# zc402/video-classification

Measured on AMD Instinct MI355X. Metric: clips/sec SlowFast-R50 8x8, 32x224^2 bf16 training step, higher is better.
Workload: dtype bf16

## Files before the change

### video-classification_amd/csrc/optim_misc.hip

```cpp
#include <string.h>

#include "sfk_common.h"

namespace {

__global__ void adam_step_inc_kernel(int64_t* step) { step[0] += 1; }

template <typename S>
__global__ __launch_bounds__(256) void adam_kernel(float* __restrict__ p, const float* __restrict__ g,
                                                   float* __restrict__ m, float* __restrict__ v, int64_t count,
                                                   float lr, float b1, float b2, float eps, float gscale,
                                                   const int64_t* step, S* __restrict__ shadow) {
  __shared__ float bc[2];
  if (threadIdx.x == 0) {
    const double t = (double)step[0];
    bc[0] = (float)(1.0 - pow((double)b1, t));
    bc[1] = (float)(1.0 - pow((double)b2, t));
  }
  __syncthreads();
  const float step_size = lr / bc[0];
  const float inv_sqrt_bc2 = 1.f / sqrtf(bc[1]);
  for (int64_t i = ((int64_t)blockIdx.x * 256 + threadIdx.x) * 4; i < count; i += (int64_t)gridDim.x * 1024) {
    if (i + 3 < count) {
      float4 pv = *reinterpret_cast<float4*>(p + i);
      const float4 gv = *reinterpret_cast<const float4*>(g + i);
      float4 mv = *reinterpret_cast<float4*>(m + i);
      float4 vv = *reinterpret_cast<float4*>(v + i);
      float* pp = reinterpret_cast<float*>(&pv);
      const float* gp = reinterpret_cast<const float*>(&gv);
      float* mp = reinterpret_cast<float*>(&mv);
      float* vp = reinterpret_cast<float*>(&vv);
#pragma unroll
      for (int j = 0; j < 4; ++j) {
        const float gj = gp[j] * gscale;
        mp[j] = b1 * mp[j] + (1.f - b1) * gj;
        vp[j] = b2 * vp[j] + (1.f - b2) * gj * gj;
        pp[j] -= step_size * mp[j] / (sqrtf(vp[j]) * inv_sqrt_bc2 + eps);
      }
      *reinterpret_cast<float4*>(p + i) = pv;
      *reinterpret_cast<float4*>(m + i) = mv;
      *reinterpret_cast<float4*>(v + i) = vv;
      if (shadow) {
#pragma unroll
        for (int j = 0; j < 4; ++j) shadow[i + j] = (S)pp[j];
      }
    } else {
      for (int64_t e = i; e < count; ++e) {
        const float gj = g[e] * gscale;
        m[e] = b1 * m[e] + (1.f - b1) * gj;
        v[e] = b2 * v[e] + (1.f - b2) * gj * gj;
        p[e] -= step_size * m[e] / (sqrtf(v[e]) * inv_sqrt_bc2 + eps);
        if (shadow) shadow[e] = (S)p[e];
      }
    }
  }
}

template <typename S, typename D>
__global__ __launch_bounds__(256) void cast_kernel(const S* __restrict__ src, D* __restrict__ dst, int64_t count) {
  for (int64_t i = (int64_t)blockIdx.x * 256 + threadIdx.x; i < count; i += (int64_t)gridDim.x * 256)
    dst[i] = (D)(float)src[i];
}

template <typename S, typename D>
__global__ __launch_bounds__(256) void filter_transpose_kernel(const S* __restrict__ src, D* __restrict__ dst,
                                                               int cout, int wtaps, int cin) {
  const int64_t total = (int64_t)cout * wtaps * cin;
  for (int64_t i = (int64_t)blockIdx.x * 256 + threadIdx.x; i < total; i += (int64_t)gridDim.x * 256) {
    const int co = (int)(i % cout);
    const int64_t r = i / cout;
    const int wi = (int)(r % wtaps);
    const int ci = (int)(r / wtaps);
    dst[i] = (D)(float)src[((int64_t)co * wtaps + wi) * cin + ci];
  }
}

template <typename D>
__global__ __launch_bounds__(256) void filter_refresh_kernel(const float* __restrict__ master, D* __restrict__ s,
                                                             D* __restrict__ st, const sfk_filter_ent* __restrict__ table,
                                                             int n) {
  __shared__ float tile[32][33];
  int lo = 0, hi = n - 1;
  const int b = blockIdx.x;
  while (lo < hi) {
    const int mid = (lo + hi + 1) >> 1;
    if (table[mid].first_block <= b) lo = mid; else hi = mid - 1;
  }
  const sfk_filter_ent e = table[lo];
  const int tiles_ci = (e.cin + 31) / 32;
  int lb = b - e.first_block;
  const int tap = lb % e.wtaps;
  lb /= e.wtaps;
  const int ci0 = (lb % tiles_ci) * 32, co0 = (lb / tiles_ci) * 32;
  const int tx = threadIdx.x & 31, ty = threadIdx.x >> 5;
#pragma unroll
  for (int i = 0; i < 4; ++i) {
    const int co = co0 + ty + 8 * i, ci = ci0 + tx;
    float v = 0.f;
    if (co < e.cout && ci < e.cin) {
      const int64_t idx = e.off + ((int64_t)co * e.wtaps + tap) * e.cin + ci;
      v = master[idx];
      if (s) s[idx] = (D)v;
    }
    tile[ty + 8 * i][tx] = v;
  }
  if (!st || !e.transpose) return;
  __syncthreads();
#pragma unroll
  for (int i = 0; i < 4; ++i) {
    const int ci = ci0 + ty + 8 * i, co = co0 + tx;
    if (co < e.cout && ci < e.cin) st[e.off + ((int64_t)ci * e.wtaps + tap) * e.cout + co] = (D)tile[tx][ty + 8 * i];
  }
}

inline unsigned grid_for(int64_t total, int per_thread = 1) {
  int64_t b = (total + 256ll * per_thread - 1) / (256ll * per_thread);
  if (b > 16384) b = 16384;
  if (b < 1) b = 1;
  return (unsigned)b;
}

}

extern "C" int sfk_adam(float* p, const float* g, float* m, float* v, int64_t count, float lr, float beta1,
                        float beta2, float eps, float grad_scale, int64_t* step, void* shadow,
                        int32_t shadow_dtype, sfk_stream_t stream) {
  if (!p || !g || !m || !v || !step || count <= 0) return SFK_ERR_INVALID;
  if ((((uintptr_t)p) | ((uintptr_t)g) | ((uintptr_t)m) | ((uintptr_t)v)) & 15) return SFK_ERR_UNSUPPORTED;
  hipStream_t s = static_cast<hipStream_t>(stream);
  hipLaunchKernelGGL(adam_step_inc_kernel, dim3(1), dim3(1), 0, s, step);
  const dim3 grid(grid_for(count, 4)), blk(256);
  if (shadow && shadow_dtype == SFK_BF16)
    hipLaunchKernelGGL(adam_kernel<bf16_t>, grid, blk, 0, s, p, g, m, v, count, lr, beta1, beta2, eps, grad_scale, step, static_cast<bf16_t*>(shadow));
  else
    hipLaunchKernelGGL(adam_kernel<float>, grid, blk, 0, s, p, g, m, v, count, lr, beta1, beta2, eps, grad_scale, step, static_cast<float*>(shadow));
  SFK_CHECK_LAUNCH();
  return SFK_OK;
}


static inline bool dtype_ok(int d) { return d == SFK_F32 || d == SFK_BF16; }

extern "C" int sfk_filter_transpose(const void* src, int32_t src_dtype, void* dst, int32_t dst_dtype, int32_t cout,
                                    int32_t wtaps, int32_t cin, sfk_stream_t stream) {
  if (!src || !dst || cout <= 0 || wtaps <= 0 || cin <= 0 || !dtype_ok(src_dtype) || !dtype_ok(dst_dtype))
    return SFK_ERR_INVALID;
  hipStream_t s = static_cast<hipStream_t>(stream);
  const int64_t total = (int64_t)cout * wtaps * cin;
  if (src_dtype == SFK_F32 && dst_dtype == SFK_F32)
    hipLaunchKernelGGL((filter_transpose_kernel<float, float>), dim3(grid_for(total)), dim3(256), 0, s, (const float*)src, (float*)dst, cout, wtaps, cin);
  else if (src_dtype == SFK_F32 && dst_dtype == SFK_BF16)
    hipLaunchKernelGGL((filter_transpose_kernel<float, bf16_t>), dim3(grid_for(total)), dim3(256), 0, s, (const float*)src, (bf16_t*)dst, cout, wtaps, cin);
  else if (src_dtype == SFK_BF16 && dst_dtype == SFK_F32)
    hipLaunchKernelGGL((filter_transpose_kernel<bf16_t, float>), dim3(grid_for(total)), dim3(256), 0, s, (const bf16_t*)src, (float*)dst, cout, wtaps, cin);
  else
    hipLaunchKernelGGL((filter_transpose_kernel<bf16_t, bf16_t>), dim3(grid_for(total)), dim3(256), 0, s, (const bf16_t*)src, (bf16_t*)dst, cout, wtaps, cin);
  SFK_CHECK_LAUNCH();
  return SFK_OK;
}

extern "C" int sfk_filter_refresh(const float* master, void* s, void* st, int32_t dtype, const sfk_filter_ent* table,
                                  int32_t n_layers, int32_t total_blocks, sfk_stream_t stream) {
  if (!master || (!s && !st) || !table || n_layers <= 0 || total_blocks <= 0 || !dtype_ok(dtype)) return SFK_ERR_INVALID;
  hipStream_t hs = static_cast<hipStream_t>(stream);
  if (dtype == SFK_BF16)
    hipLaunchKernelGGL((filter_refresh_kernel<bf16_t>), dim3((unsigned)total_blocks), dim3(256), 0, hs, master, (bf16_t*)s, (bf16_t*)st, table, n_layers);
  else
    hipLaunchKernelGGL((filter_refresh_kernel<float>), dim3((unsigned)total_blocks), dim3(256), 0, hs, master, (float*)s, (float*)st, table, n_layers);
  SFK_CHECK_LAUNCH();
  return SFK_OK;
}

extern "C" int sfk_cast(const void* src, int32_t src_dtype, void* dst, int32_t dst_dtype, int64_t count,
                        sfk_stream_t stream) {
  if (!src || !dst || count <= 0 || !dtype_ok(src_dtype) || !dtype_ok(dst_dtype)) return SFK_ERR_INVALID;
  hipStream_t s = static_cast<hipStream_t>(stream);
  if (src_dtype == SFK_F32 && dst_dtype == SFK_F32)
    hipLaunchKernelGGL((cast_kernel<float, float>), dim3(grid_for(count, 4)), dim3(256), 0, s, (const float*)src, (float*)dst, count);
  else if (src_dtype == SFK_F32 && dst_dtype == SFK_BF16)
    hipLaunchKernelGGL((cast_kernel<float, bf16_t>), dim3(grid_for(count, 4)), dim3(256), 0, s, (const float*)src, (bf16_t*)dst, count);
  else if (src_dtype == SFK_BF16 && dst_dtype == SFK_F32)
    hipLaunchKernelGGL((cast_kernel<bf16_t, float>), dim3(grid_for(count, 4)), dim3(256), 0, s, (const bf16_t*)src, (float*)dst, count);
  else
    hipLaunchKernelGGL((cast_kernel<bf16_t, bf16_t>), dim3(grid_for(count, 4)), dim3(256), 0, s, (const bf16_t*)src, (bf16_t*)dst, count);
  SFK_CHECK_LAUNCH();
  return SFK_OK;
}

extern "C" int sfk_fill_zero(void* p, size_t bytes, sfk_stream_t stream) {
  if (!p) return SFK_ERR_INVALID;
  if (bytes == 0) return SFK_OK;
  return hipMemsetAsync(p, 0, bytes, static_cast<hipStream_t>(stream)) == hipSuccess ? SFK_OK : SFK_ERR_LAUNCH;
}

namespace {
constexpr sfk_tuning kDefaults = {(uint32_t)sizeof(sfk_tuning), 5, 0, 1, 192, 256, 1, 7, 1024, 0, 48, 150, 1, 1ll << 20, 3, 512, 1, 16, 1, 3, 3};
sfk_tuning g_tuning = kDefaults;
bool g_tuning_set = false;
}
const sfk_tuning& sfk_tune() { return g_tuning; }

extern "C" int sfk_default_tuning(sfk_tuning* out) {
  if (!out || out->struct_size != sizeof(sfk_tuning)) return SFK_ERR_INVALID;
  *out = kDefaults;
  return SFK_OK;
}

extern "C" int sfk_get_tuning(sfk_tuning* out) {
  if (!out || out->struct_size != sizeof(sfk_tuning)) return SFK_ERR_INVALID;
  *out = g_tuning;
  return SFK_OK;
}

extern "C" int sfk_init(const sfk_tuning* t) {
  sfk_tuning want = kDefaults;
  if (t) {
    if (t->struct_size != sizeof(sfk_tuning)) return SFK_ERR_INVALID;
    want = *t;
  }
  if (want.bn_parts < 1 || want.wgrad_target_8w < 1 || want.wgrad_target_4w < 1 || want.pool_blocks < 1 ||
      want.igemm_short_k < 0)
    return SFK_ERR_INVALID;
  if (g_tuning_set) return memcmp(&want, &g_tuning, sizeof(want)) == 0 ? SFK_OK : SFK_ERR_INVALID;
  g_tuning = want;
  g_tuning_set = true;
  return SFK_OK;
}

extern "C" int sfk_abi_version(void) { return SFK_ABI_VERSION; }

extern "C" const char* sfk_status_string(int status) {
  switch (status) {
    case SFK_OK: return "ok";
    case SFK_ERR_INVALID: return "invalid argument";
    case SFK_ERR_UNSUPPORTED: return "unsupported shape or alignment";
    case SFK_ERR_LAUNCH: return "kernel launch failed";
    default: return "unknown status";
  }
}
```

### video-classification_amd/csrc/stem_conv.hip

```cpp
#include "sfk_common.h"

namespace {

constexpr int TS = 16;
constexpr int PR = 2 * TS + 5;
constexpr int PC = 40;
constexpr int KH = 7;

struct StemK {
  const void* src;
  int64_t sn, sc, st, sh, sw;
  int cin, t_in, h_in, w_in;
  const int32_t* t_index;
  int t_log;
  int kt, pt;
  int krows;
  int kp;
  int planes;
  int cout;
  int ho, wo, t_out;
  int tiles_h, tiles_w;
  FastDiv dtw, dth, dt, d7, dcin, dpc;
  const void* w;
  void* y;
// ... 815 lines not shown
  const int tid = threadIdx.x, lane = tid & 63, l15 = lane & 15, g = lane >> 4;
  const int wave = __builtin_amdgcn_readfirstlane(tid >> 6);
  bf16_t* yp = static_cast<bf16_t*>(k.y);
  auto a_off = [](int r, int sg) { return r * 64 + ((sg ^ ((4 - ((r >> 2) & 3)) & 3)) << 4); };
  const int perm_g = ((g & 1) << 1) | (g >> 1);
  {
    const bf16_t* wp = static_cast<const bf16_t*>(k.w);
    for (int e = tid; e < NCH * 64; e += 256) {
      const int ch = e >> 6, row = (e >> 2) & 15, gg = e & 3;
      const int cf = ch / CPF, c6 = ch % CPF;
      const int co = 16 * cf + row;
      const int kh = (c6 & 1) * 4 + (((gg & 1) << 1) | (gg >> 1)), ci = c6 >> 1;
      bf16x8 v;
#pragma unroll
      for (int i = 0; i < 8; ++i) v[i] = (bf16_t)0.f;
      if (co < k.cout && kh < KH) {
        const bf16x8 wv = *reinterpret_cast<const bf16x8*>(wp + (int64_t)co * k.kp + (ci * KH + kh) * 8);
#pragma unroll
        for (int i = 1; i < 8; ++i) v[i] = wv[i - 1];
      }
      *reinterpret_cast<bf16x8*>(amat + ch * 1024 + a_off(row, gg)) = v;
    }
  }
  __syncthreads();
  bf16x8 afr[NCH];
  {
    const int a_lane = a_off(l15, g);
#pragma unroll
    for (int ch = 0; ch < NCH; ++ch) {
      afr[ch] = *reinterpret_cast<const bf16x8*>(amat + ch * 1024 + a_lane);
      asm volatile("" : "+v"(afr[ch]));
    }
  }
  H2Stage<CIN> stg;
  stg.init(k, tid);
  uint4 xra[4], xrb[4];
  const __amdgpu_buffer_rsrc_t srs = sfk_make_rsrc(k.src, k.src_bytes);
  const __amdgpu_buffer_rsrc_t srs0 = sfk_make_rsrc(k.src, 0);
  const int b_lane = (4 * wave + perm_g) * F2_PITCH + (2 * l15 + 4) * 2;
  const int tpairs = (k.t_log + 1) / 2;
  const int tiles_h2 = (k.ho + H2_ROWS - 1) / H2_ROWS;
  H2Unit u;
  const int lb = (gridDim.x & 7) == 0 ? (int)((blockIdx.x & 7) * (gridDim.x >> 3) + (blockIdx.x >> 3)) : (int)blockIdx.x;
  for (int unit = lb; unit < nunits; unit += gridDim.x) {
    u.set(k, unit, pairs_per_unit, tchunks, tiles_h2, tpairs);
    const int n = u.n, p0 = u.p0, p1 = u.p1;
    const int ho0 = u.th2 * H2_ROWS, wo0 = u.tw * TS;
    stg.unit(k, ho0, wo0);
    const int fbase = 2 * p0;
    if (tid < 2 * (p1 - p0)) {
      const int F = fbase + tid;
      int f = (F >= 0 && F < k.t_log) ? F : -1;
      if (f >= 0 && k.t_index) f = k.t_index[f];
      fidx[tid] = (f >= 0 && f < k.t_in) ? f : -1;
    }
    __syncthreads();
    auto frame_of = [&](int F) { return __builtin_amdgcn_readfirstlane(fidx[F - fbase]); };
    stg.fetch(k, xra, srs, srs0, n, frame_of(2 * p0), frame_of(2 * p0 + 1));
    stg.stage(pb, xra);
    if (p0 + 1 < p1) stg.fetch(k, xrb, srs, srs0, n, frame_of(2 * (p0 + 1)), frame_of(2 * (p0 + 1) + 1));
    __syncthreads();
    float s1[NCF][4], s2[NCF][4];
#pragma unroll
    for (int cf = 0; cf < NCF; ++cf)
#pragma unroll
      for (int r = 0; r < 4; ++r) s1[cf][r] = s2[cf][r] = 0.f;
    auto pair_iter = [&](const int m, const int cur, uint4 (&xf)[4], const uint4 (&xs)[4]) __attribute__((always_inline)) {
      if (m + 2 < p1) stg.fetch(k, xf, srs, srs0, n, frame_of(2 * (m + 2)), frame_of(2 * (m + 2) + 1));
#pragma unroll
      for (int par = 0; par < 2; ++par) {
        const int to = 2 * m + par;
        if (to >= k.t_out) continue;
        const char* bb = pb + (cur * 2 + par) * SLOT + b_lane;
        f32x4 acc[NCF][2];
#pragma unroll
        for (int cf = 0; cf < NCF; ++cf) acc[cf][0] = acc[cf][1] = f32x4{0.f, 0.f, 0.f, 0.f};
#pragma unroll
        for (int c6 = 0; c6 < CPF; ++c6) {
          bf16x8 bv[2];
#pragma unroll
          for (int j = 0; j < 2; ++j) {
            const uint32_t* q = reinterpret_cast<const uint32_t*>(bb + (c6 >> 1) * H2_PLANE + (2 * j + 4 * (c6 & 1)) * F2_PITCH);
            uint4 t4 = make_uint4(q[0], q[1], q[2], q[3]);
            bv[j] = *reinterpret_cast<const bf16x8*>(&t4);
          }
#pragma unroll
          for (int cf = 0; cf < NCF; ++cf) {
            acc[cf][0] = __builtin_amdgcn_mfma_f32_16x16x32_bf16(afr[cf * CPF + c6], bv[0], acc[cf][0], 0, 0, 0);
            acc[cf][1] = __builtin_amdgcn_mfma_f32_16x16x32_bf16(afr[cf * CPF + c6], bv[1], acc[cf][1], 0, 0, 0);
          }
        }
        const int wo = wo0 + l15;
#pragma unroll
        for (int j = 0; j < 2; ++j) {
          const int ho = ho0 + 2 * wave + j;
          const bool pok = ho < k.ho && wo < k.wo;
          if (pok) {
#pragma unroll
            for (int cf = 0; cf < NCF; ++cf)
#pragma unroll
              for (int r = 0; r < 4; ++r) { s1[cf][r] += acc[cf][j][r]; s2[cf][r] += acc[cf][j][r] * acc[cf][j][r]; }
          }
          bf16_t* pix = yp + ((((int64_t)n * k.t_out + to) * k.ho + ho) * k.wo + wo) * k.yld + k.yoff;
#pragma unroll
          for (int cp = 0; cp < NCF; cp += 2) {
            float v[8] = {acc[cp][j][0], acc[cp][j][1], acc[cp][j][2], acc[cp][j][3],
                          acc[cp + 1][j][0], acc[cp + 1][j][1], acc[cp + 1][j][2], acc[cp + 1][j][3]};
#pragma unroll
            for (int e = 0; e < 4; ++e) stem_swap16(v[e], v[4 + e]);
            const int co = 16 * cp + 16 * (g & 1) + 8 * (g >> 1);
            if (pok && co < k.cout) {
              bf16x8 o;
#pragma unroll
              for (int e = 0; e < 8; ++e) o[e] = (bf16_t)v[e];
              *reinterpret_cast<bf16x8*>(pix + co) = o;
            }
          }
        }
      }
      if (m + 1 < p1) stg.stage(pb + (cur ^ 1) * 2 * SLOT, xs);
      __syncthreads();
    };
    for (int m = p0;;) {
      pair_iter(m, 0, xra, xrb);
      if (++m >= p1) break;
      pair_iter(m, 1, xrb, xra);
      if (++m >= p1) break;
    }
    if (k.stats) {
#pragma unroll
      for (int cf = 0; cf < NCF; ++cf)
#pragma unroll
        for (int r = 0; r < 4; ++r) {
          const float a = stem_row16_sum(s1[cf][r]), c = stem_row16_sum(s2[cf][r]);
          if (l15 == 15) {
            red[(wave * 64 + 16 * cf + 4 * g + r) * 2 + 0] = a;
            red[(wave * 64 + 16 * cf + 4 * g + r) * 2 + 1] = c;
          }
        }
      __syncthreads();
      const int half = u.th2 & 1, th = u.th2 >> 1;
      const bool alone = (u.th2 | 1) >= tiles_h2;
      const int nfr = min(2 * p1, k.t_out) - 2 * p0;
      for (int e = tid; e < nfr * k.cout; e += 256) {
        const int fr = e / k.cout, co = e - fr * k.cout;
        if (!alone && (fr & 1) != half) continue;
        float a1 = 0.f, a2 = 0.f;
        if (fr == half) {
#pragma unroll
          for (int w_ = 0; w_ < 4; ++w_) { a1 += red[(w_ * 64 + co) * 2]; a2 += red[(w_ * 64 + co) * 2 + 1]; }
        }
        const int64_t trow = (((int64_t)n * k.t_out + 2 * p0 + fr) * k.tiles_h + th) * k.tiles_w + u.tw;
        k.stats[(trow * k.cout + co) * 2 + 0] = a1;
        k.stats[(trow * k.cout + co) * 2 + 1] = a2;
      }
    }
  }
}

constexpr int V2_PC = 56;
constexpr int V2_PR = 38;
constexpr int V2_CH = 6;
constexpr int V2_DROW = 128;

__device__ __forceinline__ int v2_swz(int px) { return ((px >> 1) & 1) | (((px >> 3) & 1) << 1); }

template <int CIN>
__global__ __launch_bounds__(256, 2) void stem_wgrad_v2_kernel(const StemK k) {
  constexpr int PLANE = V2_PR * V2_PC * 2;
  constexpr int NXC = (CIN * V2_PR * V2_CH + 255) / 256;
  constexpr int NDC = 5;
  __shared__ __attribute__((aligned(16))) char smem[CIN * PLANE + 256 * V2_DROW];
  char* patch = smem;
  char* dyt = smem + CIN * PLANE;
  const int tid = threadIdx.x, lane = tid & 63, l15 = lane & 15, g = lane >> 4;
  const int wave = __builtin_amdgcn_readfirstlane(tid >> 6);
  const int lb = (gridDim.x & 7) == 0 ? (int)((blockIdx.x & 7) * (gridDim.x >> 3) + (blockIdx.x >> 3)) : (int)blockIdx.x;
  const int item0 = lb * k.tiles_per_block;
  const int item1 = min(item0 + k.tiles_per_block, k.ntiles);
  if (item0 >= item1) return;
  const bf16_t* src = static_cast<const bf16_t*>(k.src);
  const bf16_t* dyp = static_cast<const bf16_t*>(k.y);

  int x_ci[NXC], x_r[NXC], x_j[NXC];
#pragma unroll
  for (int i = 0; i < NXC; ++i) {
    const int e = tid + 256 * i;
    x_ci[i] = e / (V2_PR * V2_CH);
    const int rem = e % (V2_PR * V2_CH);
    x_r[i] = rem / V2_CH;
    x_j[i] = rem % V2_CH;
    if (e >= CIN * V2_PR * V2_CH) x_ci[i] = -1;
  }
  uint4 xr[NXC], dr[NDC];
  const __amdgpu_buffer_rsrc_t srs = sfk_make_rsrc(k.src, k.src_bytes);
  const __amdgpu_buffer_rsrc_t yrs = sfk_make_rsrc(k.y, k.y_bytes);
  const __amdgpu_buffer_rsrc_t srs0 = sfk_make_rsrc(k.src, 0);
  const __amdgpu_buffer_rsrc_t yrs0 = sfk_make_rsrc(k.y, 0);
  int x_chan[NXC];
#pragma unroll
  for (int i = 0; i < NXC; ++i) x_chan[i] = x_ci[i] < 0 ? 0 : (int)(x_ci[i] * k.sc * 2);
  auto fetch = [&](int item) {
    int n, tf, ho0, wo0;
    tile_coords(k, item, n, tf, ho0, wo0);
    int frame = k.t_index ? __builtin_amdgcn_readfirstlane(k.t_index[tf]) : tf;
    const bool fok = frame >= 0 && frame < k.t_in;
    const uint32_t xso = fok ? (uint32_t)(((int64_t)n * k.sn + (int64_t)frame * k.st) * 2) : 0u;
#pragma unroll
    for (int i = 0; i < NXC; ++i) {
      const int hi = 2 * ho0 - 3 + x_r[i], wi = 2 * wo0 - 8 + 8 * x_j[i];
      const bool ok = x_ci[i] >= 0 && (unsigned)hi < (unsigned)k.h_in && wi >= 0 && wi + 8 <= k.w_in;
      const uint32_t vo = ok ? (uint32_t)(x_chan[i] + (hi * (int)k.sh + wi) * 2) : 0x80000000u;
      const u32x4 v = __builtin_amdgcn_raw_buffer_load_b128(fok ? srs : srs0, (int)vo, (int)xso, 0);
      xr[i] = make_uint4(v[0], v[1], v[2], v[3]);
    }
    const int ho = ho0 + (tid >> 4), wo = wo0 + (tid & 15);
    const bool pok = ho < k.ho && wo < k.wo;
    const uint32_t yvo = pok ? (uint32_t)(((ho * k.wo + wo) * k.yld + k.yoff) * 2) : 0x80000000u;
    const int64_t fstride = (int64_t)k.ho * k.wo * k.yld * 2;
#pragma unroll
    for (int f = 0; f < NDC; ++f) {
      const int to = tf + k.pt - f;
      const bool ok = f < k.kt && to >= 0 && to < k.t_out;
      const uint32_t yso = ok ? (uint32_t)(((int64_t)n * k.t_out + to) * fstride) : 0u;
      const u32x4 v = __builtin_amdgcn_raw_buffer_load_b128(ok ? yrs : yrs0, (int)yvo, (int)yso, 0);
      dr[f] = make_uint4(v[0], v[1], v[2], v[3]);
    }
  };
  auto stage = [&]() {
#pragma unroll
    for (int i = 0; i < NXC; ++i)
      if (x_ci[i] >= 0)
        *reinterpret_cast<uint4*>(patch + x_ci[i] * PLANE + x_r[i] * (V2_PC * 2) + x_j[i] * 16) = xr[i];
    const int sw = v2_swz(tid);
#pragma unroll
    for (int f = 0; f < NDC; ++f)
      *reinterpret_cast<uint4*>(dyt + tid * V2_DROW + (((f >> 1) ^ sw) << 5) + (f & 1) * 16) = dr[f];
    *reinterpret_cast<uint4*>(dyt + tid * V2_DROW + ((2 ^ sw) << 5) + 16) = make_uint4(0, 0, 0, 0);
  };

  const int khh = l15 >> 3, kw = l15 & 7;
  const uint32_t sel = (kw & 1) ? 0x05040100u : 0x07060302u;
  const int cbe = (kw & 1) ? 5 + kw : 4 + kw;
  const int b_lane = ((g >> 1) * 2 + 2 * wave + khh) * (V2_PC * 2) + (2 * (g & 1) * 8 + cbe) * 2;
  const int q = l15 >> 2, p4 = lane & 3;
  int a_lane[3];
#pragma unroll
  for (int i = 0; i < 3; ++i) {
    const int row = 8 * g + q;
    a_lane[i] = row * V2_DROW + ((i ^ v2_swz(row)) << 5) + p4 * 8;
  }
  f32x4 acc[CIN][3];
#pragma unroll
  for (int c = 0; c < CIN; ++c)
#pragma unroll
    for (int i = 0; i < 3; ++i) acc[c][i] = f32x4{0.f, 0.f, 0.f, 0.f};

  fetch(item0);
  for (int item = item0; item < item1; ++item) {
    __syncthreads();
    stage();
    __syncthreads();
    if (item + 1 < item1) fetch(item + 1);
#pragma unroll
    for (int s = 0; s < 8; ++s) {
      bf16x8 a[3];
#pragma unroll
      for (int i = 0; i < 3; ++i) {
        const char* ap = dyt + s * 32 * V2_DROW + a_lane[i];
        const bf16x4 lo = __builtin_amdgcn_ds_read_tr16_b64_v4bf16((lds_bf16x4*)(ap));
        const bf16x4 hi = __builtin_amdgcn_ds_read_tr16_b64_v4bf16((lds_bf16x4*)(ap + 4 * V2_DROW));
        a[i][0] = lo[0]; a[i][1] = lo[1]; a[i][2] = lo[2]; a[i][3] = lo[3];
        a[i][4] = hi[0]; a[i][5] = hi[1]; a[i][6] = hi[2]; a[i][7] = hi[3];
      }
#pragma unroll
      for (int c = 0; c < CIN; ++c) {
        const uint32_t* bp = reinterpret_cast<const uint32_t*>(patch + c * PLANE + s * 4 * (V2_PC * 2) + b_lane);
        uint32_t d[8];
#pragma unroll
        for (int e = 0; e < 8; ++e) d[e] = bp[e];
        uint4 bv;
        bv.x = __builtin_amdgcn_perm(d[1], d[0], sel);
        bv.y = __builtin_amdgcn_perm(d[3], d[2], sel);
        bv.z = __builtin_amdgcn_perm(d[5], d[4], sel);
        bv.w = __builtin_amdgcn_perm(d[7], d[6], sel);
        const bf16x8 b = *reinterpret_cast<const bf16x8*>(&bv);
#pragma unroll
        for (int i = 0; i < 3; ++i) acc[c][i] = __builtin_amdgcn_mfma_f32_16x16x32_bf16(a[i], b, acc[c][i], 0, 0, 0);
      }
    }
  }
  const int kh = 2 * wave + khh;
  if (kh < KH && kw < 7) {
#pragma unroll
    for (int c = 0; c < CIN; ++c)
#pragma unroll
      for (int i = 0; i < 3; ++i)
#pragma unroll
        for (int r = 0; r < 4; ++r) {
          const int row = 16 * i + 4 * g + r, f = row >> 3, co = row & 7;
          if (f < k.kt && co < k.cout)
            atomicAdd(k.dw + (int64_t)co * k.kp + ((f * CIN + c) * KH + kh) * 8 + kw, acc[c][i][r]);
        }
  }
}

inline int64_t stem_src_extent(const sfk_stem_src* s, int n) {
  const int64_t esz = s->src_dtype == SFK_BF16 ? 2 : 4;
  if (s->sn < 0 || s->sc < 0 || s->st < 0 || s->sh < 0 || s->sw < 0) return (int64_t)1 << 40;
  return esz * ((int64_t)(n - 1) * s->sn + (int64_t)(s->cin - 1) * s->sc + (int64_t)(s->t_in - 1) * s->st +
                (int64_t)(s->h_in - 1) * s->sh + (int64_t)(s->w_in - 1) * s->sw + 1);
}

int fill(const sfk_stem_src* s, int cout, int t_out, int ho, int wo, StemK& k) {
  if (!s || !s->src || s->cin <= 0 || s->kt <= 0 || !(s->kt & 1) || s->t_in <= 0 || s->h_in <= 0 || s->w_in <= 0)
    return SFK_ERR_INVALID;
  if (s->src_dtype != SFK_F32 && s->src_dtype != SFK_BF16) return SFK_ERR_INVALID;
  const int t_log = s->t_index ? s->t_len : s->t_in;
  if (t_log <= 0 || t_out != t_log) return SFK_ERR_INVALID;
  if (ho != (s->h_in + 6 - 7) / 2 + 1 || wo != (s->w_in + 6 - 7) / 2 + 1) return SFK_ERR_INVALID;
  if (cout <= 0 || cout > 64 || (cout % 4)) return SFK_ERR_UNSUPPORTED;
  k.src = s->src; k.sn = s->sn; k.sc = s->sc; k.st = s->st; k.sh = s->sh; k.sw = s->sw;
  k.cin = s->cin; k.t_in = s->t_in; k.h_in = s->h_in; k.w_in = s->w_in; k.t_index = s->t_index; k.t_log = t_log;
  k.kt = s->kt; k.pt = s->kt / 2;
  k.planes = s->kt * s->cin;
  k.krows = k.planes * KH;
  k.kp = ((k.krows + 3) / 4) * 4 * 8;
  k.cout = cout; k.ho = ho; k.wo = wo; k.t_out = t_out;
  k.tiles_h = (ho + TS - 1) / TS; k.tiles_w = (wo + TS - 1) / TS;
  k.dtw.set(k.tiles_w); k.dth.set(k.tiles_h); k.dt.set(t_out); k.d7.set(KH); k.dcin.set(s->cin); k.dpc.set(PC);
  k.lut = nullptr; k.crop = nullptr; k.pad = 0;
  return SFK_OK;
}

int fill_u8(const sfk_u8_clip* x, const int32_t* t_index, int32_t t_len, int32_t kt, int n, int cout, int t_out, int ho,
            int wo, StemK& k) {
  if (!sfk_u8_clip_ok(x) || x->n != n) return SFK_ERR_INVALID;
  sfk_stem_src s{};
  s.src = x->src + x->c0;
  s.src_dtype = SFK_F32;
  s.sn = x->sn; s.sc = 1; s.st = x->st; s.sh = x->sh; s.sw = x->sw;
  s.cin = x->c; s.t_in = x->t; s.h_in = x->h; s.w_in = x->w;
  s.t_index = t_index; s.t_len = t_len; s.kt = kt;
  const int st = fill(&s, cout, t_out, ho, wo, k);
  if (st != SFK_OK) return st;
  k.lut = x->lut; k.crop = x->crop; k.pad = x->pad;
  return SFK_OK;
}

template <typename S>
int stem_fwd_generic(StemK& k, const sfk_fmap* y, hipStream_t hs) {
  const int fn = (y->c + 15) / 16;
  const size_t esz = y->dtype == SFK_BF16 ? 2 : 4;
  const size_t lds = esz * ((size_t)16 * fn * (k.kp + 8) + (size_t)k.planes * PR * PC) + 4 * 16 * fn * 2 * sizeof(float) +
                     (sfk_is_u8<S> ? 256 * sizeof(float) : 0);
  if (lds > 160 * 1024) return SFK_ERR_UNSUPPORTED;
  k.ntiles = y->n * y->t * k.tiles_h * k.tiles_w;
  const int resident = 256 * (int)((160 * 1024) / lds < 1 ? 1 : ((160 * 1024) / lds > 4 ? 4 : (160 * 1024) / lds));
  const dim3 grid((unsigned)(k.ntiles < 4 * resident ? k.ntiles : 4 * resident)), blk(256);
#define SFK_STEM_FWD(T, FN)                                                                                 \
  do {                                                                                                      \
    if (lds > 64 * 1024)                                                                                    \
      (void)hipFuncSetAttribute(reinterpret_cast<const void*>(&stem_fwd_kernel<T, S, FN>),                      \
                          hipFuncAttributeMaxDynamicSharedMemorySize, (int)lds);                            \
    hipLaunchKernelGGL((stem_fwd_kernel<T, S, FN>), grid, blk, lds, hs, k);                                 \
  } while (0)
#define SFK_STEM_FWD_FN(T)                                          \
  do {                                                              \
    if (fn == 1) SFK_STEM_FWD(T, 1);                                \
    else if (fn == 2) SFK_STEM_FWD(T, 2);                           \
    else SFK_STEM_FWD(T, 4);                                        \
  } while (0)
  if (fn == 3) return SFK_ERR_UNSUPPORTED;
  if (y->dtype == SFK_BF16) SFK_STEM_FWD_FN(bf16_t);
  else SFK_STEM_FWD_FN(float);
#undef SFK_STEM_FWD_FN
#undef SFK_STEM_FWD
  SFK_CHECK_LAUNCH();
  return SFK_OK;
}

template <typename S>
int stem_wgrad_generic(StemK& k, const sfk_fmap* dy, hipStream_t hs) {
  int splits = (2048 + k.planes - 1) / k.planes;
  if (splits > k.ntiles) splits = k.ntiles;
  if (splits > 65535) splits = 65535;
  k.tiles_per_block = (k.ntiles + splits - 1) / splits;
  splits = (k.ntiles + k.tiles_per_block - 1) / k.tiles_per_block;
  const int fn = (dy->c + 15) / 16;
  if (fn == 3) return SFK_ERR_UNSUPPORTED;
  const dim3 grid((unsigned)k.planes, (unsigned)splits), blk(256);
#define SFK_STEM_WG(T)                                                                      \
  do {                                                                                      \
    if (fn == 1) hipLaunchKernelGGL((stem_wgrad_kernel<T, S, 1>), grid, blk, 0, hs, k);     \
    else if (fn == 2) hipLaunchKernelGGL((stem_wgrad_kernel<T, S, 2>), grid, blk, 0, hs, k); \
    else hipLaunchKernelGGL((stem_wgrad_kernel<T, S, 4>), grid, blk, 0, hs, k);             \
  } while (0)
  if (dy->dtype == SFK_BF16) SFK_STEM_WG(bf16_t);
  else SFK_STEM_WG(float);
#undef SFK_STEM_WG
  SFK_CHECK_LAUNCH();
  return SFK_OK;
}

}

extern "C" int sfk_stem_kp(int32_t cin, int32_t kt) { return ((kt * cin * KH + 3) / 4) * 4 * 8; }

extern "C" int sfk_stem_conv_tiles(const sfk_stem_src* s, const sfk_fmap* y) {
  if (!s || !sfk_fmap_ok(y)) return SFK_ERR_INVALID;
  return y->n * y->t * ((y->h + TS - 1) / TS) * ((y->w + TS - 1) / TS);
}

extern "C" int sfk_stem_conv_fwd(const sfk_stem_src* s, const void* w, const sfk_fmap* y, float* stats,
                                 sfk_stream_t stream) {
  if (!w || !sfk_fmap_ok(y)) return SFK_ERR_INVALID;
  StemK k;
  const int st = fill(s, y->c, y->t, y->h, y->w, k);
  if (st != SFK_OK) return st;
  if ((y->ld % 4) || (y->c_off % 4) || (((uintptr_t)y->ptr) & 15) || (((uintptr_t)w) & 15)) return SFK_ERR_UNSUPPORTED;
  k.w = w; k.y = y->ptr; k.yld = y->ld; k.yoff = y->c_off; k.stats = stats; k.dw = nullptr;
  k.ntiles = y->n * y->t * k.tiles_h * k.tiles_w;
  if (y->dtype == SFK_BF16 && s->src_dtype == SFK_BF16 && s->cin == 3 && (s->kt == 5 || s->kt == 3) && y->c <= 8 &&
      s->sw == 1 && (s->w_in % 8) == 0 && !((s->sn | s->sc | s->st | s->sh) & 7) && !(((uintptr_t)s->src) & 15) &&
      stem_src_extent(s, y->n) < (1ll << 32) - 64) {
    k.src_bytes = (uint32_t)stem_src_extent(s, y->n);
    k.y_bytes = 0;
    hipStream_t hs2 = static_cast<hipStream_t>(stream);
    const int nf = s->kt + 1;
    const int lds2 = nf * 3 * F2_PLANE + nf * 6 * 1024 + 8 * 16 * 2 * 4;
    const int tpairs = (k.t_log + 1) / 2;
    const int ppu = tpairs < 8 ? tpairs : 8;
    const int nunits = y->n * k.tiles_h * k.tiles_w * ((tpairs + ppu - 1) / ppu);
    const int grid2 = nunits < 256 ? nunits : 256;
    const bool v3 = (sfk_tune().stem_v3 & 1) != 0 && stem_src_extent(s, y->n) < (1ll << 31) && k.t_log >= 2;
    if (v3) {
      const int nfull = k.t_log / 2, tch = nfull <= ppu ? 1 : (nfull + ppu - 1) / ppu;
      const int nu = y->n * ((y->h + H2_ROWS - 1) / H2_ROWS) * k.tiles_w * tch;
      const int grid4 = nu < 512 ? nu : 512;
      const int lds4 = 4 * 3 * H2_PLANE + nf * 6 * 1024 + 4 * 16 * 2 * 4 + 32 * 4;
      if (s->kt == 5) {
        (void)hipFuncSetAttribute(reinterpret_cast<const void*>(&stem_fwd_v4_kernel<3, 5>), hipFuncAttributeMaxDynamicSharedMemorySize, lds4);
        hipLaunchKernelGGL((stem_fwd_v4_kernel<3, 5>), dim3((unsigned)grid4), dim3(256), lds4, hs2, k, ppu, nu, tch);
      } else {
        (void)hipFuncSetAttribute(reinterpret_cast<const void*>(&stem_fwd_v4_kernel<3, 3>), hipFuncAttributeMaxDynamicSharedMemorySize, lds4);
        hipLaunchKernelGGL((stem_fwd_v4_kernel<3, 3>), dim3((unsigned)grid4), dim3(256), lds4, hs2, k, ppu, nu, tch);
      }
    } else if (s->kt == 5) {
      (void)hipFuncSetAttribute(reinterpret_cast<const void*>(&stem_fwd_v2_kernel<3, 5>), hipFuncAttributeMaxDynamicSharedMemorySize, lds2);
      hipLaunchKernelGGL((stem_fwd_v2_kernel<3, 5>), dim3((unsigned)grid2), dim3(512), lds2, hs2, k, ppu, nunits);
    } else {
      (void)hipFuncSetAttribute(reinterpret_cast<const void*>(&stem_fwd_v2_kernel<3, 3>), hipFuncAttributeMaxDynamicSharedMemorySize, lds2);
      hipLaunchKernelGGL((stem_fwd_v2_kernel<3, 3>), dim3((unsigned)grid2), dim3(512), lds2, hs2, k, ppu, nunits);
    }
    SFK_CHECK_LAUNCH();
    return SFK_OK;
  }
  if ((sfk_tune().stem_v3 & 2) && y->dtype == SFK_BF16 && s->src_dtype == SFK_BF16 && s->cin == 3 && s->kt == 1 && y->c == 64 &&
      s->sw == 1 && (s->w_in % 8) == 0 && !((s->sn | s->sc | s->st | s->sh) & 7) && !(((uintptr_t)s->src) & 15) &&
      !(y->ld % 8) && !(y->c_off % 8) && stem_src_extent(s, y->n) < (1ll << 31) && k.t_log >= 2) {
    k.src_bytes = (uint32_t)stem_src_extent(s, y->n);
    k.y_bytes = 0;
    hipStream_t hs3 = static_cast<hipStream_t>(stream);
    const int ppu = 2;
    const int nfull = k.t_log / 2, tch = nfull <= ppu ? 1 : (nfull + ppu - 1) / ppu;
    const int nu = y->n * ((y->h + H2_ROWS - 1) / H2_ROWS) * k.tiles_w * tch;
    const int grid4 = nu < 512 ? nu : 512;
    const int lds4 = 4 * 3 * H2_PLANE + 24 * 1024 + 4 * 64 * 2 * 4 + 32 * 4;
    (void)hipFuncSetAttribute(reinterpret_cast<const void*>(&stem_fwd_s4_kernel<3>), hipFuncAttributeMaxDynamicSharedMemorySize, lds4);
    hipLaunchKernelGGL((stem_fwd_s4_kernel<3>), dim3((unsigned)grid4), dim3(256), lds4, hs3, k, ppu, nu, tch);
    SFK_CHECK_LAUNCH();
    return SFK_OK;
  }
  hipStream_t hs = static_cast<hipStream_t>(stream);
  return s->src_dtype == SFK_BF16 ? stem_fwd_generic<bf16_t>(k, y, hs) : stem_fwd_generic<float>(k, y, hs);
}

extern "C" int sfk_stem_conv_wgrad(const sfk_stem_src* s, const sfk_fmap* dy, float* dw, sfk_stream_t stream) {
  if (!dw || !sfk_fmap_ok(dy)) return SFK_ERR_INVALID;
  StemK k;
  const int st = fill(s, dy->c, dy->t, dy->h, dy->w, k);
  if (st != SFK_OK) return st;
  if (!sfk_fmap_vec_ok(dy)) return SFK_ERR_UNSUPPORTED;
  k.w = nullptr; k.y = dy->ptr; k.yld = dy->ld; k.yoff = dy->c_off; k.stats = nullptr; k.dw = dw;
  k.ntiles = dy->n * dy->t * k.tiles_h * k.tiles_w;
  hipStream_t hs = static_cast<hipStream_t>(stream);
  if (dy->dtype == SFK_BF16 && s->src_dtype == SFK_BF16 && s->cin == 3 && s->kt <= 5 && dy->c <= 8 && s->sw == 1 &&
      (s->w_in % 8) == 0 && !((s->sn | s->sc | s->st | s->sh) & 7) && !(((uintptr_t)s->src) & 15) &&
      stem_src_extent(s, dy->n) < (1ll << 31) && sfk_fmap_bytes(dy) < (1ll << 31)) {
    k.src_bytes = (uint32_t)stem_src_extent(s, dy->n);
    k.y_bytes = (uint32_t)sfk_fmap_bytes(dy);
    int blocks = 256 * 3;
    if (blocks > k.ntiles) blocks = k.ntiles;
    k.tiles_per_block = (k.ntiles + blocks - 1) / blocks;
    blocks = (k.ntiles + k.tiles_per_block - 1) / k.tiles_per_block;
    blocks = (blocks + 7) & ~7;
    hipLaunchKernelGGL((stem_wgrad_v2_kernel<3>), dim3((unsigned)blocks), dim3(256), 0, hs, k);
    SFK_CHECK_LAUNCH();
    return SFK_OK;
  }
  return s->src_dtype == SFK_BF16 ? stem_wgrad_generic<bf16_t>(k, dy, hs) : stem_wgrad_generic<float>(k, dy, hs);
}

extern "C" int sfk_u8stem_abi_version(void) { return SFK_U8STEM_ABI_VERSION; }

extern "C" int sfk_u8stem_conv_fwd(const sfk_u8_clip* x, const int32_t* t_index, int32_t t_len, int32_t kt, const void* w,
                                   const sfk_fmap* y, float* stats, sfk_stream_t stream) {
  if (!w || !sfk_fmap_ok(y)) return SFK_ERR_INVALID;
  StemK k;
  const int st = fill_u8(x, t_index, t_len, kt, y->n, y->c, y->t, y->h, y->w, k);
  if (st != SFK_OK) return st;
  if ((y->ld % 4) || (y->c_off % 4) || (((uintptr_t)y->ptr) & 15) || (((uintptr_t)w) & 15)) return SFK_ERR_UNSUPPORTED;
  k.w = w; k.y = y->ptr; k.yld = y->ld; k.yoff = y->c_off; k.stats = stats; k.dw = nullptr;
  hipStream_t hs = static_cast<hipStream_t>(stream);
  if (x->c == 5) return stem_fwd_generic<U8Pix<5>>(k, y, hs);
  if (x->c == 15) return stem_fwd_generic<U8Pix<15>>(k, y, hs);
  return stem_fwd_generic<U8Lut>(k, y, hs);
}

extern "C" int sfk_u8stem_conv_wgrad(const sfk_u8_clip* x, const int32_t* t_index, int32_t t_len, int32_t kt,
                                     const sfk_fmap* dy, float* dw, sfk_stream_t stream) {
  if (!dw || !sfk_fmap_ok(dy)) return SFK_ERR_INVALID;
  StemK k;
  const int st = fill_u8(x, t_index, t_len, kt, dy->n, dy->c, dy->t, dy->h, dy->w, k);
  if (st != SFK_OK) return st;
  if (!sfk_fmap_vec_ok(dy)) return SFK_ERR_UNSUPPORTED;
  k.w = nullptr; k.y = dy->ptr; k.yld = dy->ld; k.yoff = dy->c_off; k.stats = nullptr; k.dw = dw;
  k.ntiles = dy->n * dy->t * k.tiles_h * k.tiles_w;
  return stem_wgrad_generic<U8Lut>(k, dy, static_cast<hipStream_t>(stream));
}
```

Baseline: 1156.

## Add v3 stem weight-gradient kernel with temporal ring and cross-wave reduction

Adds a new stem-conv weight-gradient kernel that splits the work across waves along the kernel-row and batch dimensions. It keeps a five-slot temporal ring of dy tiles in LDS, prefetches the next frame's input and dy into registers while computing the current one, and sums partial accumulators across waves in shared memory before issuing one set of atomicAdds per block. This is meant to cut atomic traffic and improve reuse across frames. It also accepts half-width (4-channel) dy layouts and is enabled by default through a tuning bit. Tiles per block rise to at least eight, which may reduce parallelism.

```diff
diff --git a/video-classification_amd/csrc/optim_misc.hip b/video-classification_amd/csrc/optim_misc.hip
--- a/video-classification_amd/csrc/optim_misc.hip
+++ b/video-classification_amd/csrc/optim_misc.hip
@@ -194,7 +194,7 @@
 }
 
 namespace {
-constexpr sfk_tuning kDefaults = {(uint32_t)sizeof(sfk_tuning), 5, 0, 1, 192, 256, 1, 7, 1024, 0, 48, 150, 1, 1ll << 20, 3, 512, 1, 16, 1, 3, 3};
+constexpr sfk_tuning kDefaults = {(uint32_t)sizeof(sfk_tuning), 5, 0, 1, 192, 256, 1, 7, 1024, 0, 48, 150, 1, 1ll << 20, 3, 512, 1, 16, 1, 3, 7};
 sfk_tuning g_tuning = kDefaults;
 bool g_tuning_set = false;
 }
diff --git a/video-classification_amd/csrc/stem_conv.hip b/video-classification_amd/csrc/stem_conv.hip
--- a/video-classification_amd/csrc/stem_conv.hip
+++ b/video-classification_amd/csrc/stem_conv.hip
@@ -1141,6 +1141,212 @@
           if (f < k.kt && co < k.cout)
             atomicAdd(k.dw + (int64_t)co * k.kp + ((f * CIN + c) * KH + kh) * 8 + kw, acc[c][i][r]);
         }
+  }
+}
+
+constexpr int V3_ZSLOT = 7;
+constexpr int V3_MIN_ITEMS = 8;
+constexpr int V3_BLOCKS = 512;
+
+constexpr int V3_EP = 64;
+constexpr int V3_ODD = V2_PR * V3_EP + 32;
+constexpr int V3_CPL = 2 * V2_PR * V3_EP + 64;
+
+template <int CIN>
+__global__ __launch_bounds__(256, 2) void stem_wgrad_v3_kernel(const StemK k) {
+  constexpr int PITCH = V3_EP, PLANE = V3_CPL;
+  constexpr int NXC = (CIN * V2_PR * V2_CH + 255) / 256;
+  constexpr int NCF = 4;
+  constexpr int NFR = CIN * NCF * 3;
+  constexpr int LDS = CIN * PLANE + 256 * V2_DROW;
+  static_assert(NFR * 64 * 16 <= LDS, "the cross-wave sum reuses the staging buffers");
+  static_assert(NFR % 4 == 0, "the flush splits the fragments over four waves");
+  __shared__ __attribute__((aligned(16))) char smem[LDS];
+  char* patch = smem;
+  char* dyt = smem + CIN * PLANE;
+  const int tid = threadIdx.x, lane = tid & 63, l15 = lane & 15, g = lane >> 4;
+  const int wave = __builtin_amdgcn_readfirstlane(tid >> 6);
+  const int lb = (gridDim.x & 7) == 0 ? (int)((blockIdx.x & 7) * (gridDim.x >> 3) + (blockIdx.x >> 3)) : (int)blockIdx.x;
+  const int item0 = lb * k.tiles_per_block;
+  const int item1 = min(item0 + k.tiles_per_block, k.ntiles);
+  if (item0 >= item1) return;
+
+  int x_ci[NXC], x_r[NXC], x_j[NXC], x_chan[NXC];
+#pragma unroll
+  for (int i = 0; i < NXC; ++i) {
+    const int e = tid + 256 * i;
+    x_ci[i] = e / (V2_PR * V2_CH);
+    const int rem = e % (V2_PR * V2_CH);
+    x_r[i] = rem / V2_CH;
+    x_j[i] = rem % V2_CH;
+    if (e >= CIN * V2_PR * V2_CH) x_ci[i] = -1;
+    x_chan[i] = x_ci[i] < 0 ? 0 : (int)(x_ci[i] * k.sc * 2);
+  }
+  uint4 xr[NXC], dr;
+  const __amdgpu_buffer_rsrc_t srs = sfk_make_rsrc(k.src, k.src_bytes);
+  const __amdgpu_buffer_rsrc_t yrs = sfk_make_rsrc(k.y, k.y_bytes);
+  const int lead = k.kt - 1;
+  const int64_t fstride = (int64_t)k.ho * k.wo * k.yld * 2;
+
+  struct Pos { int n, ho0, wo0, tfa, tfb, tf, next; };
+  auto open = [&](int item, Pos& p) {
+    uint32_t col, tf0, q1, tw, n_, th;
+    k.dt.divmod((uint32_t)item, col, tf0);
+    k.dtw.divmod(col, q1, tw);
+    k.dth.divmod(q1, n_, th);
+    p.n = (int)n_; p.ho0 = (int)th * TS; p.wo0 = (int)tw * TS;
+    p.tfa = (int)tf0;
+    p.tfb = min(k.t_log, p.tfa + (item1 - item));
+    p.next = item + (p.tfb - p.tfa);
+    p.tf = p.tfa - lead;
+  };
+  auto advance = [&](Pos& p) -> bool {
+    if (++p.tf < p.tfb) return true;
+    if (p.next >= item1) return false;
+    open(p.next, p);
+    return true;
+  };
+  auto fetch = [&](const Pos& p, bool valid, uint4 (&xs)[NXC], uint4& ds) {
+    {
+      const bool live = valid && p.tf >= p.tfa;
+      const int tfc = __builtin_amdgcn_readfirstlane(min(max(p.tf, 0), k.t_log - 1));
+      const int frame = k.t_index ? reinterpret_cast<const __attribute__((address_space(4))) int32_t*>((uintptr_t)k.t_index)[tfc] : tfc;
+      const bool fok = live && frame >= 0 && frame < k.t_in;
+      const uint32_t xso = (uint32_t)__builtin_amdgcn_readfirstlane((int)(fok ? (uint32_t)(((int64_t)p.n * k.sn + (int64_t)frame * k.st) * 2) : 0u));
+#pragma unroll
+      for (int i = 0; i < NXC; ++i) {
+        const int hi = 2 * p.ho0 - 3 + x_r[i], wi = 2 * p.wo0 - 8 + 8 * x_j[i];
+        const bool ok = fok && x_ci[i] >= 0 && (unsigned)hi < (unsigned)k.h_in && wi >= 0 && wi + 8 <= k.w_in;
+        const uint32_t vo = ok ? (uint32_t)(x_chan[i] + (hi * (int)k.sh + wi) * 2) : 0x80000000u;
+        const u32x4 v = __builtin_amdgcn_raw_buffer_load_b128(srs, (int)vo, (int)xso, 0);
+        xs[i] = make_uint4(v[0], v[1], v[2], v[3]);
+      }
+    }
+    const int ho = p.ho0 + (tid >> 4), wo = p.wo0 + (tid & 15);
+    const int to = p.tf + k.pt;
+    const bool ok = valid && to >= 0 && to < k.t_out;
+    const bool pok = ok && ho < k.ho && wo < k.wo;
+    const uint32_t yvo = pok ? (uint32_t)(((ho * k.wo + wo) * k.yld + k.yoff) * 2) : 0x80000000u;
+    const uint32_t yso = (uint32_t)__builtin_amdgcn_readfirstlane((int)(ok ? (uint32_t)(((int64_t)p.n * k.t_out + to) * fstride) : 0u));
+    const u32x4 v = __builtin_amdgcn_raw_buffer_load_b128(yrs, (int)yvo, (int)yso, 0);
+    ds = make_uint4(v[0], v[1], v[2], v[3]);
+  };
+  const int st_sw = v2_swz(tid) << 1;
+  auto stage = [&](const Pos& p, const uint4 (&xs)[NXC], const uint4& ds) {
+    if (p.tf >= p.tfa) {
+#pragma unroll
+      for (int i = 0; i < NXC; ++i)
+        if (x_ci[i] >= 0) {
+          char* ep = patch + x_ci[i] * PLANE + x_r[i] * PITCH + x_j[i] * 8;
+          *reinterpret_cast<uint2*>(ep) = make_uint2(__builtin_amdgcn_perm(xs[i].y, xs[i].x, 0x05040100u),
+                                                     __builtin_amdgcn_perm(xs[i].w, xs[i].z, 0x05040100u));
+          *reinterpret_cast<uint2*>(ep + V3_ODD) = make_uint2(__builtin_amdgcn_perm(xs[i].y, xs[i].x, 0x07060302u),
+                                                              __builtin_amdgcn_perm(xs[i].w, xs[i].z, 0x07060302u));
+        }
+    }
+    const int slot = (p.tf + k.pt + 10) % 5;
+    *reinterpret_cast<uint4*>(dyt + tid * V2_DROW + ((slot ^ st_sw) << 4)) = ds;
+  };
+  *reinterpret_cast<uint4*>(dyt + tid * V2_DROW + ((V3_ZSLOT ^ st_sw) << 4)) = make_uint4(0, 0, 0, 0);
+
+  const int kpart = wave & 1, npart = wave >> 1;
+  const int khh = l15 >> 3, kw = l15 & 7;
+  const int x0 = 8 * (g & 1) + ((kw + 5) >> 1);
+  const uint32_t bsh = (x0 & 1) * 16;
+  const int b_base = ((g >> 1) * 2 + khh + 16 * kpart + 4 * npart) * PITCH + ((kw & 1) ? 0 : V3_ODD) + (x0 >> 1) * 4;
+  const int q = l15 >> 2, p4 = lane & 3;
+  const int a_row = (128 * kpart + 8 * g + q) * V2_DROW + (p4 & 1) * 8;
+  const int a_sw = v2_swz(8 * g + q) << 1;
+  f32x4 acc[CIN][2][3];
+#pragma unroll
+  for (int c = 0; c < CIN; ++c)
+#pragma unroll
+    for (int cf = 0; cf < 2; ++cf)
+#pragma unroll
+      for (int i = 0; i < 3; ++i) acc[c][cf][i] = f32x4{0.f, 0.f, 0.f, 0.f};
+  auto compute = [&](const Pos& p) __attribute__((always_inline)) {
+    int a_off[3];
+#pragma unroll
+    for (int i = 0; i < 3; ++i) {
+      const int s0 = 2 * i < k.kt ? (p.tf + k.pt - 2 * i + 10) % 5 : V3_ZSLOT;
+      const int s1 = 2 * i + 1 < k.kt ? (p.tf + k.pt - 2 * i - 1 + 10) % 5 : V3_ZSLOT;
+      a_off[i] = a_row + ((((p4 >> 1) ? s1 : s0) ^ a_sw) << 4);
+    }
+#pragma unroll
+    for (int ss = 0; ss < 4; ++ss) {
+      bf16x8 a[3];
+#pragma unroll
+      for (int i = 0; i < 3; ++i) {
+        const char* ap = dyt + ss * 32 * V2_DROW + a_off[i];
+        const bf16x4 lo = __builtin_amdgcn_ds_read_tr16_b64_v4bf16((lds_bf16x4*)(ap));
+        const bf16x4 hi = __builtin_amdgcn_ds_read_tr16_b64_v4bf16((lds_bf16x4*)(ap + 4 * V2_DROW));
+        a[i][0] = lo[0]; a[i][1] = lo[1]; a[i][2] = lo[2]; a[i][3] = lo[3];
+        a[i][4] = hi[0]; a[i][5] = hi[1]; a[i][6] = hi[2]; a[i][7] = hi[3];
+      }
+#pragma unroll
+      for (int c = 0; c < CIN; ++c)
+#pragma unroll
+        for (int cf = 0; cf < 2; ++cf) {
+          const uint32_t* bp = reinterpret_cast<const uint32_t*>(patch + c * PLANE + (4 * ss + 2 * cf) * PITCH + b_base);
+          uint32_t d[5];
+#pragma unroll
+          for (int e = 0; e < 5; ++e) d[e] = bp[e];
+          uint4 bv;
+          bv.x = __builtin_amdgcn_alignbit(d[1], d[0], bsh);
+          bv.y = __builtin_amdgcn_alignbit(d[2], d[1], bsh);
+          bv.z = __builtin_amdgcn_alignbit(d[3], d[2], bsh);
+          bv.w = __builtin_amdgcn_alignbit(d[4], d[3], bsh);
+          const bf16x8 b = *reinterpret_cast<const bf16x8*>(&bv);
+#pragma unroll
+          for (int i = 0; i < 3; ++i) acc[c][cf][i] = __builtin_amdgcn_mfma_f32_16x16x32_bf16(a[i], b, acc[c][cf][i], 0, 0, 0);
+        }
+    }
+  };
+
+  Pos cur, ahead;
+  open(item0, cur);
+  ahead = cur;
+  fetch(cur, true, xr, dr);
+  bool more = advance(ahead);
+  for (bool go = true; go;) {
+    __syncthreads();
+    stage(cur, xr, dr);
+    __syncthreads();
+    fetch(ahead, more, xr, dr);
+    if (more) more = advance(ahead);
+    if (cur.tf >= cur.tfa) compute(cur);
+    go = advance(cur);
+  }
+  f32x4* red = reinterpret_cast<f32x4*>(smem);
+#pragma unroll 1
+  for (int w = 0; w < 2; ++w) {
+    __syncthreads();
+    if (kpart == w) {
+#pragma unroll
+      for (int c = 0; c < CIN; ++c)
+#pragma unroll
+        for (int cf = 0; cf < 2; ++cf)
+#pragma unroll
+          for (int i = 0; i < 3; ++i) {
+            f32x4* rp = red + ((c * NCF + 2 * npart + cf) * 3 + i) * 64 + lane;
+            *rp = w == 0 ? acc[c][cf][i] : *rp + acc[c][cf][i];
+          }
+    }
+  }
+  __syncthreads();
+#pragma unroll 1
+  for (int j = 0; j < NFR / 4; ++j) {
+    const int fr = wave * (NFR / 4) + j;
+    const int i = fr % 3, cc = fr / 3, cf = cc % NCF, c = cc / NCF;
+    const int kh = 2 * cf + khh;
+    if (kh >= KH || kw >= 7) continue;
+    const f32x4 v = red[fr * 64 + lane];
+#pragma unroll
+    for (int r = 0; r < 4; ++r) {
+      const int row = 16 * i + 4 * g + r, f = row >> 3, co = row & 7;
+      if (f < k.kt && co < k.cout)
+        atomicAdd(k.dw + (int64_t)co * k.kp + ((f * CIN + c) * KH + kh) * 8 + kw, v[r]);
+    }
   }
 }
 
@@ -1320,15 +1526,26 @@
   StemK k;
   const int st = fill(s, dy->c, dy->t, dy->h, dy->w, k);
   if (st != SFK_OK) return st;
-  if (!sfk_fmap_vec_ok(dy)) return SFK_ERR_UNSUPPORTED;
+  const bool fast = dy->dtype == SFK_BF16 && s->src_dtype == SFK_BF16 && s->cin == 3 && s->kt <= 5 && dy->c <= 8 && s->sw == 1 &&
+      (s->w_in % 8) == 0 && !((s->sn | s->sc | s->st | s->sh) & 7) && !(((uintptr_t)s->src) & 15) &&
+      stem_src_extent(s, dy->n) < (1ll << 31) && sfk_fmap_bytes(dy) < (1ll << 31);
+  const bool half = fast && dy->c == 4 && !(dy->ld % 4) && !(dy->c_off % 4) && !(((uintptr_t)dy->ptr) & 15);
+  if (!sfk_fmap_vec_ok(dy) && !half) return SFK_ERR_UNSUPPORTED;
   k.w = nullptr; k.y = dy->ptr; k.yld = dy->ld; k.yoff = dy->c_off; k.stats = nullptr; k.dw = dw;
   k.ntiles = dy->n * dy->t * k.tiles_h * k.tiles_w;
   hipStream_t hs = static_cast<hipStream_t>(stream);
-  if (dy->dtype == SFK_BF16 && s->src_dtype == SFK_BF16 && s->cin == 3 && s->kt <= 5 && dy->c <= 8 && s->sw == 1 &&
-      (s->w_in % 8) == 0 && !((s->sn | s->sc | s->st | s->sh) & 7) && !(((uintptr_t)s->src) & 15) &&
-      stem_src_extent(s, dy->n) < (1ll << 31) && sfk_fmap_bytes(dy) < (1ll << 31)) {
+  if (fast) {
     k.src_bytes = (uint32_t)stem_src_extent(s, dy->n);
     k.y_bytes = (uint32_t)sfk_fmap_bytes(dy);
+    if (sfk_tune().stem_v3 & 4) {
+      int per = (k.ntiles + V3_BLOCKS - 1) / V3_BLOCKS;
+      if (per < V3_MIN_ITEMS) per = V3_MIN_ITEMS;
+      k.tiles_per_block = per;
+      const int nb = (((k.ntiles + per - 1) / per) + 7) & ~7;
+      hipLaunchKernelGGL((stem_wgrad_v3_kernel<3>), dim3((unsigned)nb), dim3(256), 0, hs, k);
+      SFK_CHECK_LAUNCH();
+      return SFK_OK;
+    }
     int blocks = 256 * 3;
     if (blocks > k.ntiles) blocks = k.ntiles;
     k.tiles_per_block = (k.ntiles + blocks - 1) / blocks;
```

Result: no change. 1161 (median of 6 runs) (+0.5%).
